# Plachtaa/FAcodec

Measured on AMD Instinct MI355X. Metric: 24kHz audio sec encoded+decoded per wall-sec, higher is better.
Workload: dtype f32; 1 GPU; configs[1]: batch=32/GPU x 2 s @ 24 kHz, forward encoder->FVQ(6 codebooks)->decoder, FAcodec configs/config.yml model (137.7 M params), weights formula-generated, weight-norm re-materialised every step; clips_per_gpu=32, samples_per_clip=48000, parallelism=dp1 (independent clips, no collective)

## Files before the change

### facodec_amd/_lib.py

```python
import ctypes as C
import os

_HERE = os.path.dirname(os.path.abspath(__file__))
LIB_PATH = os.environ.get("FAC_LIB_PATH", os.path.join(_HERE, "libfacodec_hip.so"))

PAD_ZERO, PAD_REFLECT = 0, 1
ACT_NONE, ACT_TANH, ACT_MISH, ACT_LOG_MEL = 0, 1, 2, 3
ACT_GATE, ACT_WN_RES_SKIP = 4, 5

_p = C.c_void_p
_i = C.c_int
_i64 = C.c_int64
_f = C.c_float


class ConvDesc(C.Structure):
    _fields_ = [
        ("x", _p), ("w", _p), ("bias", _p), ("alpha_in", _p), ("alpha_out", _p), ("res", _p), ("y", _p), ("y2", _p), ("alpha_y2", _p), ("w_k1", _p), ("bias_k1", _p),
        ("x_bs", _i64), ("x_cs", _i64), ("y_bs", _i64), ("y_cs", _i64),
        ("B", C.c_int32), ("C_in", C.c_int32), ("T_in", C.c_int32), ("C_out", C.c_int32),
        ("C_out_pad", C.c_int32), ("T_out", C.c_int32),
        ("K", C.c_int32), ("stride", C.c_int32), ("dilation", C.c_int32), ("pad_left", C.c_int32),
        ("pad_mode", C.c_int32), ("n_phase", C.c_int32), ("y_tstride", C.c_int32), ("phase_shift", C.c_int32),
        ("act", C.c_int32),
# ... 211 lines not shown
    "fac_glu_residual": (_i, [_p, _p, _p, _i, _i, _i, _p]),
    "fac_add": (_i, [_p, _p, _p, _i64, _p]),
    "fac_sub2": (_i, [_p, _p, _p, _p, _i64, _p]),
    "fac_mul_mask": (_i, [_p, _p, _i, _i, _i, _p]),
    "fac_wn_res_skip": (_i, [_p, _p, _p, _i, _i, _i, _i, _p]),
    "fac_attention": (_i, [_p, _p, _p, _p, _p, _i, _i, _i, _i, _p]),
    "fac_attention_stream": (_i, [_p, _p, _p, _p, _p, _i, _i, _i, _i, _p]),
    "fac_attention_route": (_i, [_i, _i]),
    "fac_attention_form": (_i, [_i, _i]),
    "fac_attention_tiled_fits": (_i, [_i, _i]),
    "fac_attention_tiled": (_i, [_p, _p, _p, _p, _p, _i, _i, _i, _i, _p]),
    "fac_attention_serial": (_i, [_p, _p, _p, _p, _p, _i, _i, _i, _i, _p]),
    "fac_attention_stream_tile": (_i, [_i]),
    "fac_masked_mean": (_i, [_p, _p, _p, _i, _i, _i, _p]),
    "fac_layernorm_c_affine": (_i, [_p, _p, _p, _i, _i, _i, _p]),
    "fac_stft_frames": (_i, [_p, _p, _i, _i, _i, _i, _i, _i, _i, _p]),
    "fac_stft_frames_ragged": (_i, [_p, _p, _p, _i, _i, _i, _i, _i, _i, _i, _p]),
    "fac_mask_tail": (_i, [_p, _p, _i, _i, _i, _i, _p]),
    "fac_mask_tail_i64": (_i, [_p, _p, _i, _i, _i, _i, _p]),
    "fac_edge_tail": (_i, [_p, _p, _i, _i, _i, _i, _i, _i, _p]),
    "fac_frame_mask": (_i, [_p, _p, _p, _i, _i, _i, _p]),
    "fac_resample": (_i, [C.POINTER(ResampleDesc), _p]),
    "fac_resample_form": (_i, [C.POINTER(ResampleDesc), _p]),
    "fac_kweight_ws_bytes": (_i64, [_i, _i]),
    "fac_kweight_energy": (_i, [C.POINTER(KweightDesc), _p]),
    "fac_loudness_chunk": (_i, [_i]),
    "fac_loudness_gate": (_i, [_p, _i64, _p, _i64, _i, _i, _p, _i, _p, _p, _i, _p]),
    "fac_loudness_gain": (_i, [_p, _i64, _p, _p, _p, _p, C.c_double, _i, _p, _i64, _p, _i, _i, _p]),
    "fac_si_sdr_ws_bytes": (_i64, [_i, _i]),
    "fac_si_sdr": (_i, [_p, _i64, _p, _i64, _p, _p, _p, _i64, _i, _i, _p]),
# ... 49 lines not shown
```

### facodec_amd/csrc/common.h

```cpp
#pragma once
#include <hip/hip_runtime.h>
#include <stdint.h>
#include <stdio.h>
#include <stdarg.h>
#include "../../include/facodec_hip.h"

namespace fac {

void set_error(const char* fmt, ...);

inline int check_launch(const char* what) {
  hipError_t e = hipGetLastError();
  if (e != hipSuccess) {
    set_error("%s: launch failed: %s", what, hipGetErrorString(e));
    return FAC_ERR_LAUNCH;
  }
  return FAC_OK;
}

#define FAC_REQUIRE(cond, ...)          \
  do {                                  \
    if (!(cond)) {                      \
      ::fac::set_error(__VA_ARGS__);    \
      return FAC_ERR_ARG;               \
// ... 57 lines not shown
}
__device__ __forceinline__ f32x2 snake_apply2(f32x2 x, float alpha, float inv) { return x + inv * sin_sq2(alpha * x); }

__device__ __attribute__((noinline)) float apply_act_slow(float v, int act) {
  if (act == FAC_ACT_TANH) return tanhf(v);
  if (act == FAC_ACT_MISH) {
    const float sp = v > 20.f ? v : log1pf(expf(v));
    return v * tanhf(sp);
  }
  if (act == FAC_ACT_LOG_MEL) return (logf(1e-5f + v) + 4.0f) / 4.0f;
  return v;
}

__device__ __forceinline__ float sigmoid_f(float x) { return __fdiv_rn(1.0f, 1.0f + expf(-x)); }

__device__ __forceinline__ int reflect_index(int t, int T, int Text) {
  int j;
  if (t < 0) j = -t;
  else if (t < Text) j = t;
  else j = 2 * (Text - 1) - t;
  return (j >= 0 && j < T) ? j : -1;
}


typedef __bf16 bf16x8 __attribute__((ext_vector_type(8)));
typedef __bf16 bf16x4 __attribute__((ext_vector_type(4)));
typedef float f32x16 __attribute__((ext_vector_type(16)));
typedef float f32x4 __attribute__((ext_vector_type(4)));
typedef unsigned u32x4 __attribute__((ext_vector_type(4)));

// ... 76 lines not shown
```

### facodec_amd/csrc/conv1d_api.hip

```cpp
#include "conv1d_mfma.h"
#include <stdlib.h>

namespace fac {

enum ConvKernel : int {
  CK_128x32 = 0,
  CK_32x256 = 1,
  CK_64x128 = 2,
  CK_96x128 = 3,
  CK_128x128 = 4,
  CK_128x256 = 5,
  CK_96x256 = 6,
  CK_FUSED_RU = 7,
  CK_128x160 = 8,
  CK_NARROW = 9,
  CK_SKINNY = 10,
  CK_BSPLIT = 11,
  CK_CIN1 = 12,
  CK_THIN = 13,
  CK_PW = 14,
  CK_GSPLIT = 15,
  CK_BSPLIT2 = 16,
  CK_PWS = 17,
  CK_PWT = 18,
// ... 73 lines not shown
  {
    long long last = (long long)(d->T_out - 1) * d->stride + (long long)conv_max_tap_offset(a) - d->pad_left;
    int pad_right = last >= d->T_in ? (int)(last - d->T_in + 1) : 0;
    int max_pad = d->pad_left > pad_right ? d->pad_left : pad_right;
    a.T_ext = d->T_in > max_pad ? d->T_in : max_pad + 1;
  }
  if (d->x_p8 || d->y2_p8) {
    const bool gs = d->w_split && (d->K <= 2 || (d->stride > 1 && d->K <= 2 * d->stride)) && conv_gsplit_ok(a) &&
                    !conv_skinny_ok(a, d->ws, d->ws_bytes) && d->C_in % 8 == 0 && d->x_p8_plane_bytes < (1ll << 32);
    const bool ok = !d->y2_p8 && (gs || (d->w_split && !conv_two_level(a) && (d->split_rows == 96 ? conv_bsplit96_p8_ok(a) : conv_bsplit_p8_ok(a)) &&
                                       !conv_cin1_ok(a)));
    FAC_REQUIRE(ok, "conv1d: P8 operands given but the launch does not run on a kernel that takes them (K=%d stride=%d C_in=%d columns=%lld)",
                d->K, d->stride, d->C_in, (long long)d->B * d->T_out);
  }
  if (d->act == FAC_ACT_GATE || d->act == FAC_ACT_WN_RES_SKIP) {
    FAC_REQUIRE(d->w && !d->w_k1 && !d->x_p8 && !conv_two_level(a) && conv_skinny_ok(a, d->ws, d->ws_bytes),
                "conv1d: FAC_ACT_GATE / FAC_ACT_WN_RES_SKIP exist only for few-column launches (B * T_out <= 640) with a workspace");
    k = CK_SKINNY;
    return FAC_OK;
  }
  if (d->w_k1) { k = CK_FUSED_RU; return FAC_OK; }
  a.gflat = 0;
  a.grt = 0;
  if (d->w_split && (a.KV == 9 || a.KV == 3) && d->C_out <= 32 && conv_bsplit2_ok(a)) {
    a.w = reinterpret_cast<const float*>(d->w_split);
    k = CK_BSPLIT2;
    return FAC_OK;
  }
  FAC_REQUIRE(!conv_two_level(a) || d->w, "conv1d: two-level taps outside the split kernel's shapes need fp32 weights");
  const bool pw_on = pw_enabled();
  if (pw_on && d->pw_split && d->w && conv_pwt_ok(a)) { k = CK_PWT; return FAC_OK; }
  if (d->w_split && (d->K <= 2 || (d->stride > 1 && d->K <= 2 * d->stride)) && conv_gsplit_ok(a) &&
      !conv_skinny_ok(a, d->ws, d->ws_bytes)) {
    a.w = reinterpret_cast<const float*>(d->w_split);
    k = CK_GSPLIT;
// ... 108 lines not shown
```

### facodec_amd/csrc/conv1d_bsplit.hip

```cpp
#include "conv1d_bsplit_kernel.h"

namespace fac {

__device__ __forceinline__ void pack_conv_split_body(const float* __restrict__ v, const float* __restrict__ scale,
                                                     bf16x8* __restrict__ out, int C_out, int C_in, int K, int G, int H, int n_st,
                                                     int CO, long long n, int vb, int vg) {
  for (long long idx = (long long)vb * 256 + threadIdx.x; idx < n; idx += (long long)vg * 256) {
    const int co = (int)(idx % CO);
    long long r = idx / CO;
    const int hs = (int)(r % H);
    r /= H;
    const int s = (int)(r % n_st);
    const int ct = (int)(r / n_st);
    const int g = hs % G, k = hs / G;
    const int cog = ct * CO + co;
    const float sc = (scale != nullptr && cog < C_out) ? scale[cog] : 1.0f;
    bf16x8 h, m, l;
#pragma unroll
    for (int i = 0; i < 8; ++i) {
      const int ci = (s * G + g) * 8 + i;
      float w = 0.f;
      if (cog < C_out && ci < C_in && k < K) {
        w = v[((long long)cog * C_in + ci) * K + k];
        if (scale != nullptr) w = __fmul_rn(w, sc);
      }
      __bf16 a, b2, c;
      split3(w, a, b2, c);
      h[i] = a; m[i] = b2; l[i] = c;
    }
    const long long base = ((long long)ct * n_st + s) * 3;
    out[((base + 0) * H + hs) * CO + co] = h;
    out[((base + 1) * H + hs) * CO + co] = m;
    out[((base + 2) * H + hs) * CO + co] = l;
  }
}

__global__ __launch_bounds__(256) void pack_conv_split_kernel(const float* __restrict__ v, const float* __restrict__ scale,
                                                              bf16x8* __restrict__ out, int C_out, int C_in, int K, int G, int H,
                                                              int n_st, int CO, long long n) {
  pack_conv_split_body(v, scale, out, C_out, C_in, K, G, H, n_st, CO, n, blockIdx.x, gridDim.x);
}

__global__ __launch_bounds__(256) void bsplit_batch_kernel(const PrepJob* __restrict__ jobs, const int* __restrict__ first, int njobs) {
  const int j = prep_find_job(first, njobs, blockIdx.x);
  const PrepJob& J = jobs[j];
  pack_conv_split_body(static_cast<const float*>(J.a), static_cast<const float*>(J.b), static_cast<bf16x8*>(J.out), J.i[0], J.i[1],
                       J.i[2], J.i[3], J.i[4], J.i[5], J.i[6], J.n, blockIdx.x - first[j], J.nblocks);
}

int prep_launch_bsplit(const PrepJob* jobs, const int* first, int njobs, int total, hipStream_t s) {
  hipLaunchKernelGGL(bsplit_batch_kernel, dim3(total), dim3(256), 0, s, jobs, first, njobs);
  return check_launch("bsplit_batch");
}

bool conv_bsplit_ok(const ConvArgs& a) {
  if (!((a.K == 7 || a.K == 5 || a.K == 3) && a.stride == 1 && a.n_phase == 1 && a.phase_shift == 0 && a.y_tstride == 1 && !a.alpha_in &&
        !a.w1 && !a.w_batched && (long long)a.B * a.T_out > 640))
    return false;
  const int G = bs_group(a.C_in), tt = G == 2 ? 256 : 512;
  const int kp = G == 2 ? a.K - 1 : ((a.K + 1) & ~1) - 1;
  return a.C_in % (8 * G) == 0 && G * ((tt + kp * a.dil + 63) / 64) <= BS_NSW * BS_XU &&
         a.x_cs * (long long)a.C_in < (1ll << 31);
// ... 13 lines not shown

}

extern "C" int fac_debug_bsplit_occupancy(int lds_bytes) {
  int n = -1;
  auto kern = fac::conv1d_bsplit_kernel<7, 2, 4, fac::BS_NSW_WIDE>;
  (void)hipFuncSetAttribute(reinterpret_cast<const void*>(kern), hipFuncAttributeMaxDynamicSharedMemorySize, (int)fac::FAC_LDS_MAX);
  if (hipOccupancyMaxActiveBlocksPerMultiprocessor(&n, kern, (4 + fac::BS_NSW) * 64, (size_t)lds_bytes) != hipSuccess) return -1;
  return n;
}

static bool split_rows_ok(int K, int rows) { return rows == fac::BS_CO || (rows == fac::BS96_CO && K == 7); }

extern "C" int64_t fac_conv_w_split_rows_bytes(int C_out, int C_in, int K, int rows) {
  using namespace fac;
  if (!split_rows_ok(K, rows)) return -1;
  const int G = rows == BS96_CO ? 1 : bs_group(C_in);
  const int64_t n_ct = (C_out + rows - 1) / rows, n_st = (C_in + 8 * G - 1) / (8 * G);
  return n_ct * n_st * 3 * bs_slots(K, G) * rows * 16;
}

extern "C" int64_t fac_conv_w_split_bytes(int C_out, int C_in, int K) { return fac_conv_w_split_rows_bytes(C_out, C_in, K, fac::BS_CO); }

extern "C" int fac_pack_conv_w_split_rows(const float* v, const float* scale, void* out, int C_out, int C_in, int K, int rows,
                                          fac_stream_t stream) {
  using namespace fac;
  FAC_REQUIRE(v && out && C_out > 0 && C_in > 0 && K > 0, "pack_conv_w_split: bad arguments");
  FAC_REQUIRE(split_rows_ok(K, rows), "pack_conv_w_split: no %d-row tile for K=%d", rows, K);
  const int G = rows == BS96_CO ? 1 : bs_group(C_in);
  const int n_ct = (C_out + rows - 1) / rows, n_st = (C_in + 8 * G - 1) / (8 * G), H = bs_slots(K, G);
  const long long n = (long long)n_ct * n_st * H * rows;
  const int blocks = (int)((n + 255) / 256 < 65535 ? (n + 255) / 256 : 65535);
  if (prep_recording()) {
    PrepJob j{}; j.a = v; j.b = scale; j.out = out; j.kind = PK_CONV_SPLIT; j.nblocks = blocks; j.n = n;
    j.i[0] = C_out; j.i[1] = C_in; j.i[2] = K; j.i[3] = G; j.i[4] = H; j.i[5] = n_st; j.i[6] = rows;
    return prep_record(PU_BSPLIT, j);
  }
  hipLaunchKernelGGL(pack_conv_split_kernel, dim3(blocks), dim3(256), 0, (hipStream_t)stream, v, scale,
                     reinterpret_cast<bf16x8*>(out), C_out, C_in, K, G, H, n_st, rows, n);
  return check_launch("pack_conv_w_split");
}

extern "C" int fac_pack_conv_w_split(const float* v, const float* scale, void* out, int C_out, int C_in, int K,
                                     fac_stream_t stream) {
  return fac_pack_conv_w_split_rows(v, scale, out, C_out, C_in, K, fac::BS_CO, stream);
}
```

### facodec_amd/csrc/conv1d_bsplit_kernel.h

```cpp
#pragma once
#include "conv1d_mfma.h"
#include <type_traits>
#include "inflight_regs.h"
#include "prep_batch.h"

namespace fac {

constexpr int BS_CO = 64;
constexpr int BS96_CO = 96;
constexpr int BS_NSW = 4;
constexpr int BS_NSW_WIDE = 4;
constexpr int BS_XU = 3;
constexpr int BS_WIDE_MIN = 64;
__host__ __device__ constexpr int bs_group(int C_in) { return C_in >= BS_WIDE_MIN ? 2 : 1; }

__host__ __device__ constexpr int bs_slots(int K, int G) { return (G * K + 1) & ~1; }

struct EpiRow {
  float bs, al, inv, a2, i2;
};
__device__ __forceinline__ EpiRow epi_row_load(bool valid, int co, const float* bias, const float* alpha, const float* alpha2) {
  EpiRow r = {0.f, 0.f, 0.f, 0.f, 0.f};
  if (valid) {
    if (bias) r.bs = bias[co];
// ... 448 lines not shown
  {
    const KArgP e = fresh_args();
    const float* tile = reinterpret_cast<const float*>(epi_base);
    constexpr int EP = BS_TT + 4;
    constexpr int NTH = (NMW + NSW) * 64;
    constexpr int QPR = BS_TT / 4;
    float* yg = e->y ? e->y + (long long)b * e->y_bs : nullptr;
    float* y2g = e->y2 ? e->y2 + (long long)b * e->y_bs : nullptr;
    const float* rg = e->res ? e->res + (long long)b * e->y_bs : nullptr;
    const bool vec_ok = (e->y_cs & 3) == 0 && (e->y_bs & 3) == 0 && (!yg || (reinterpret_cast<unsigned long long>(e->y) & 15) == 0) &&
                        (!y2g || (reinterpret_cast<unsigned long long>(e->y2) & 15) == 0) &&
                        (!rg || (reinterpret_cast<unsigned long long>(e->res) & 15) == 0);
    static_assert(QPR % 16 == 0 && NTH % 16 == 0 && (CO * QPR) % 64 == 0 && (CO * QPR + NTH - 1) / NTH <= 16, "EpiRow: 16 lanes share a row, <= 16 iterations");
    const int row_l = (tid + NTH * (lane & 15)) / QPR;
    const EpiRow mine = epi_row_load(row_l < CO && co0 + row_l < e->C_out, co0 + row_l, e->bias, e->alpha_out, y2g ? e->alpha2 : nullptr);
    int j = 0;
    for (int q = tid; q < CO * QPR; q += NTH, ++j) {
      const float bs = epi_row_get(mine.bs, lane, j), al = epi_row_get(mine.al, lane, j), inv = epi_row_get(mine.inv, lane, j);
      float a2 = 0.f, i2 = 0.f;
      if (y2g) { a2 = epi_row_get(mine.a2, lane, j); i2 = epi_row_get(mine.i2, lane, j); }
      const int row = q / QPR, tq = q - row * QPR;
      const int co = co0 + row, t = t0 + 4 * tq;
      if (co >= e->C_out || t >= e->T_out) continue;
      const float4 av = *reinterpret_cast<const float4*>(tile + row * EP + 4 * tq);
      f32x2 v[2] = {{av.x, av.y}, {av.z, av.w}};
      const long long o = (long long)co * e->y_cs + t;
      const bool full = vec_ok && t + 3 < e->T_out;
      float rv[4] = {0.f, 0.f, 0.f, 0.f};
      if (rg) {
        if (full) {
// ... 16 lines not shown
#pragma unroll
        for (int i = 0; i < 2; ++i) w[i] = snake_apply2(v[i], a2, i2);
      }
      if (full) {
        if (yg) *reinterpret_cast<float4*>(yg + o) = make_float4(v[0].x, v[0].y, v[1].x, v[1].y);
        if (y2g) *reinterpret_cast<float4*>(y2g + o) = make_float4(w[0].x, w[0].y, w[1].x, w[1].y);
      } else {
#pragma unroll
        for (int i = 0; i < 4; ++i) {
          if (t + i >= e->T_out) continue;
          if (yg) yg[o + i] = v[i >> 1][i & 1];
          if (y2g) y2g[o + i] = w[i >> 1][i & 1];
        }
      }
    }
  }
  first = !overlap;
  if (vb + (int)gridDim.x < n_tiles) __syncthreads();
  }
  };
  if (wave >= NMW) {
    if constexpr (WIDE) {
      if (a.x_p8 != nullptr) walk(std::integral_constant<int, 2>{});
      else walk(std::integral_constant<int, 1>{});
    } else {
      walk(std::integral_constant<int, 1>{});
    }
  } else {
    walk(std::integral_constant<int, 0>{});
  }
// ... 32 lines not shown
```

### facodec_amd/csrc/misc.hip

```cpp
#include "common.h"
#include <string.h>

namespace fac {

static thread_local char g_err[512] = "";

void set_error(const char* fmt, ...) {
  va_list ap;
  va_start(ap, fmt);
  vsnprintf(g_err, sizeof(g_err), fmt, ap);
  va_end(ap);
}

constexpr int EW_THREADS = 256;
inline int ew_grid(long long n, int per_thread = 1) {
  long long g = (n + (long long)EW_THREADS * per_thread - 1) / ((long long)EW_THREADS * per_thread);
  if (g > 8192) g = 8192;
  if (g < 1) g = 1;
  return (int)g;
}

__global__ void snake_kernel(const float* __restrict__ x, const float* __restrict__ alpha,
                             float* __restrict__ y, int C, int T, long long n) {
  for (long long i = (long long)blockIdx.x * blockDim.x + threadIdx.x; i < n;
// ... 307 lines not shown
  if (tv) {
    const float var = ((red[1][0][lane] + red[1][1][lane]) + (red[1][2][lane] + red[1][3][lane])) / (float)C;
    rstd = __fdiv_rn(1.0f, sqrtf(var + 1e-5f));
    if (wave == 0) {
      stat[0][lane] = mean;
      stat[1][lane] = rstd;
    }
  }
  __syncthreads();
  const float* gm = style + (long long)b * 2 * C;
  float* ob = out + (long long)b * C * T;
  for (int i = tid; i < C * T; i += 256) {
    const int c = i / T, tt = i - c * T;
    const float nv = __fmul_rn(xs[i] - stat[0][tt], stat[1][tt]);
    ob[i] = __fadd_rn(__fmul_rn(nv, gm[c]), gm[C + c]);
  }
}

__global__ void stft_frames_kernel(const float* __restrict__ wave, float* __restrict__ frames, int T,
                                   int n_win, int n_frames, int hop, int pad, int n_off,
                                   long long n) {
  const long long per_b = (long long)n_win * n_frames;
  for (long long i = (long long)blockIdx.x * blockDim.x + threadIdx.x; i < n;
       i += (long long)gridDim.x * blockDim.x) {
    const long long b = i / per_b;
    const long long r = i - b * per_b;
    const int nn = (int)(r / n_frames);
    const int f = (int)(r - (long long)nn * n_frames);
    int t = f * hop + nn + n_off - pad;
    if (t < 0) t = -t;
// ... 218 lines not shown
    const float k = r > 0.f ? scale / ((float)M * r) : 0.f;
    for (int m = 0; m < M; ++m) {
      const float bv = pb[(long long)m * T];
      const float d = logf(fabsf(pa[(long long)m * T]) + eps) - logf(fabsf(bv) + eps);
      const float sg = bv > 0.f ? 1.f : (bv < 0.f ? -1.f : 0.f);
      const float g = -k * d * sg / (fabsf(bv) + eps);
      pd[(long long)m * T] = accumulate ? pd[(long long)m * T] + g : g;
    }
  }
}

}

using namespace fac;

extern "C" int fac_version(void) { return 5; }
extern "C" const char* fac_last_error(void) { return fac::g_err; }

#define EW_LAUNCH(kern, n, ...)                                                         \
  hipLaunchKernelGGL(kern, dim3(ew_grid(n)), dim3(EW_THREADS), 0, (hipStream_t)stream, __VA_ARGS__)

extern "C" int fac_snake_fwd(const float* x, const float* alpha, float* y, int B, int C, int T,
                             fac_stream_t stream) {
  FAC_REQUIRE(x && alpha && y && B > 0 && C > 0 && T > 0, "snake_fwd: bad arguments");
  const long long n = (long long)B * C * T;
  if (T >= 1024 && (long long)B * C <= 65535) {
    hipLaunchKernelGGL(snake_rows_kernel, dim3((T + 1023) / 1024, B * C), dim3(256), 0, (hipStream_t)stream, x, alpha, y, C, T);
  } else {
    EW_LAUNCH(snake_kernel, n, x, alpha, y, C, T, n);
  }
  return check_launch("snake_fwd");
// ... 92 lines not shown
  if (stage_v) lds = lds_v;
  allow_dynamic_lds<attention_kernel>();
  dim3 grid((T + 15) / 16, n_heads, B);
  hipLaunchKernelGGL(attention_kernel, grid, dim3(256), lds, (hipStream_t)stream, q, k, v, mask, out,
                     n_heads, dk, T, stage_v);
  return check_launch("attention");
}

extern "C" int fac_masked_mean(const float* x, const float* mask, float* out, int B, int C, int T,
                               fac_stream_t stream) {
  FAC_REQUIRE(x && out && B > 0 && C > 0 && T > 0, "masked_mean: bad arguments");
  hipLaunchKernelGGL(masked_mean_kernel, dim3(C, B), dim3(64), 0, (hipStream_t)stream, x, mask, out, C, T);
  return check_launch("masked_mean");
}

extern "C" int fac_layernorm_c_affine(const float* x, const float* style, float* out, int B, int C,
                                      int T, fac_stream_t stream) {
  FAC_REQUIRE(x && style && out && B > 0 && C > 0 && T > 0, "layernorm_c_affine: bad arguments");
  if (T <= 8 && (size_t)C * T * 4 <= 64 * 1024) {
    hipLaunchKernelGGL(layernorm_c_small_t_kernel, dim3(B), dim3(256), (size_t)C * T * 4, (hipStream_t)stream, x,
                       style, out, C, T);
    return check_launch("layernorm_c_affine(small T)");
  }
  hipLaunchKernelGGL(layernorm_c_kernel, dim3((T + 63) / 64, B), dim3(256), 0, (hipStream_t)stream, x,
                     style, out, C, T);
  return check_launch("layernorm_c_affine");
}

extern "C" int fac_stft_frames(const float* wave, float* frames, int B, int T, int n_win,
                               int n_frames, int hop, int pad, int n_off, fac_stream_t stream) {
  FAC_REQUIRE(wave && frames && B > 0 && T > 0 && n_win > 0 && n_frames > 0 && hop > 0,
              "stft_frames: bad arguments");
  FAC_REQUIRE(pad < T, "stft_frames: reflect pad %d needs a signal longer than %d samples", pad, T);
  const long long n = (long long)B * n_win * n_frames;
  EW_LAUNCH(stft_frames_kernel, n, wave, frames, T, n_win, n_frames, hop, pad, n_off, n);
  return check_launch("stft_frames");
}

extern "C" int fac_spec_power(const float* spec, float* out, int B, int F, int n_frames, int power,
                              fac_stream_t stream) {
  FAC_REQUIRE(spec && out && B > 0 && F > 0 && n_frames > 0 && (power == 1 || power == 2),
// ... 120 lines not shown
```

### facodec_amd/layers.py

```python
import math

import torch
from torch import nn

from . import ops


def _uniform_(t, bound):
    with torch.no_grad():
        return t.uniform_(-bound, bound)


class ConvWeights(nn.Module):

    def __init__(self, c_in, c_out, k, weight_norm=True, transposed=False, stride=1, bias=True):
        super().__init__()
        self.c_in, self.c_out, self.k = c_in, c_out, k
        self.transposed, self.stride, self.weight_norm = transposed, stride, weight_norm
        shape = (c_in, c_out, k) if transposed else (c_out, c_in, k)
        fan_in = (c_out if transposed else c_in) * k
        w = _uniform_(torch.empty(shape), 1.0 / math.sqrt(fan_in))
        if weight_norm:
            self.weight_g = nn.Parameter(w.reshape(shape[0], -1).norm(dim=1).reshape(shape[0], 1, 1))
            self.weight_v = nn.Parameter(w)
        else:
            self.weight = nn.Parameter(w)
        self.bias = nn.Parameter(_uniform_(torch.empty(c_out), 1.0 / math.sqrt(fan_in))) if bias else None
        self._packed = None
        self._split = None
        self._rows = None
        self._rows_split = None
        self.freeze_packed = False

    def _vg(self):
        return (self.weight_v.detach(), self.weight_g.detach()) if self.weight_norm else (self.weight.detach(), None)

    def _cached(self, slot, pack, *a, **kw):
        cur = getattr(self, slot)
        if cur is None or not self.freeze_packed:
            cur = pack(*self._vg(), *a, out=cur[0] if isinstance(cur, tuple) else cur, **kw)
            setattr(self, slot, cur)
        return cur

    def packed(self):
# ... 1 lines not shown
            return self._cached("_packed", ops.pack_convtr_weight, self.stride)
        return self._cached("_packed", ops.pack_conv_weight)

    def packed_rows(self):
        return self._cached("_rows", ops.pack_convtr_weight_rows, self.stride)

    def packed_rows_split(self):
        return self._cached("_rows_split", ops.pack_convtr_weight_rows_split, self.stride)

    def packed_split_strided(self, stride):
        return self._cached("_split", ops.pack_gemm_weight_split, in_stride=stride)

    def packed_split(self, rows=64):
        return self._cached("_split", ops.pack_conv_weight_split, rows=rows)

    def _apply(self, fn, *a, **kw):
        self._packed = None
        self._split = None
        self._rows = None
        self._rows_split = None
        return super()._apply(fn, *a, **kw)


class _Norm(nn.Module):

    def __init__(self, name, weights):
        super().__init__()
        setattr(self, name, weights)


FLAT_SHORT_CLIPS = True
FLAT_STRIDE1 = True

# ... 21 lines not shown
    def plan(self, B, T, alpha_in=False, plain=True, res=False):
        return ops.plan_conv(self.w.c_out, self.w.c_in, self.kernel_size, self.stride, self.dilation, B, T, -(-T // self.stride),
                             alpha_in=alpha_in, plain=plain, res=res, causal_reflect=self.causal and self.pad_mode == ops.PAD_REFLECT,
                             grad=torch.is_grad_enabled(), c_out_mult16=False, tail="always", flat_infer=FLAT_SHORT_CLIPS,
                             flat_stride1=FLAT_STRIDE1)

    def edge_rule(self):
        if self.causal:
            return None
        if self.stride != 1:
            raise NotImplementedError(f"a non-causal strided SConv1d (k = {self.kernel_size}, stride {self.stride}) pads its right "
                                      "side by an amount that depends on the clip's length: no per-clip edge rule")
        n = ((self.kernel_size - 1) * self.dilation) // 2
        return (n, self.pad_mode) if n > 0 else None

    def run(self, x, alpha_in=None, alpha_out=None, res=None, act=ops.ACT_NONE, alpha_y2=None, want_y=True, edge=None):
        w, k, s_ = self.w, self.kernel_size, self.stride
        write_edge(self, x, edge)
        B, _, T = x.shape
        plan = self.plan(B, T, alpha_in is not None, alpha_out is None and res is None and act == ops.ACT_NONE, res is not None)
        split = (w.packed_split_strided(s_) if plan.layout == ops.W_GEMM_STRIDED
                 else w.packed_split(ops.tile_rows(w.c_out, w.c_in, k)) if plan.layout == ops.W_TAPS
                 else w.packed_split() if plan.layout == ops.W_GEMM else None)
        if plan.form != ops.PER_CLIP:
            P = (k - 1) * self.dilation + 1 - s_
            return ops.conv1d_flat(torch.nn.functional.pad(x, (P, 0), mode="reflect"), split, w.c_out, k, s_, T // s_,
                                   dilation=self.dilation, bias=w.bias, p8=plan.p8, alpha_out=alpha_out, act=act, alpha_y2=alpha_y2,
                                   want_y=want_y)
        x = ops.p8_prepass(x, plan.p8)
        return ops.conv1d(x, w.packed() if split is None else None, w.c_out, k, bias=w.bias,
                          stride=s_, dilation=self.dilation, pad_mode=self.pad_mode, alpha_in=alpha_in,
                          alpha_out=alpha_out, res=res, act=act, causal=self.causal, alpha_y2=alpha_y2, want_y=want_y,
                          w_split=split)

    def forward(self, x):
        return self.run(x)


class SConvTranspose1d(nn.Module):

    def __init__(self, in_channels, out_channels, kernel_size, stride=1, causal=False, norm="none"):
        super().__init__()
        self.convtr = _Norm("convtr", ConvWeights(in_channels, out_channels, kernel_size, norm == "weight_norm",
                                                  transposed=True, stride=stride))
        self.stride = stride
        self.causal = causal

    @property
# ... 79 lines not shown
```

### facodec_amd/ops.py

```python
import ctypes as C
import math
import os
from collections import namedtuple

import torch

from . import _lib
from .wprep import prepared
from .convplan import *
from ._lib import ConvDesc, VqDesc, VqDecodeDesc, ResampleDesc, PAD_REFLECT, PAD_ZERO, ACT_NONE, ACT_TANH, ACT_MISH, ACT_LOG_MEL, ACT_GATE, ACT_WN_RES_SKIP


def pad32(n):
    return (n + 31) & ~31


def cin_pad(c):
    return ((c + 47) // 48) * 48


_RAW_STREAM = getattr(torch._C, "_cuda_getCurrentRawStream", None)
_GET_DEVICE = getattr(torch._C, "_cuda_getDevice", None)


# ... 341 lines not shown
    return out


@prepared
def pack_convtr_weight_rows_split(v, g, stride, out=None):
    rows = pack_convtr_weight_rows(v, g, stride)
    cip, _, R = rows.shape
    c_in = v.shape[0]
    lib = _lib.load()
    nbytes = lib.fac_gemm_w_split_bytes(R, c_in, 2, 1)
    if out is None:
        out = torch.empty(nbytes, device=v.device, dtype=torch.uint8)
    _lib.check(lib.fac_pack_gemm_w_split(_ptr(rows), 1, 2 * R, R, None, out.data_ptr(), R, c_in, 2, 1, _stream()),
               "fac_pack_gemm_w_split(convtr rows)")
    return out, R


@prepared
def pack_conv_weight_split(v, g=None, out=None, scale=None, rows=None):
    v = _dev(v, "weight")
    c_out, c_in, k = v.shape
    if k <= 2:
        return pack_gemm_weight_split(v, g, out=out, scale=scale)
    lib = _lib.load()
    if scale is None and g is not None:
        scale = wn_scale(v, g)
    if rows is None:
        rows = tile_rows(c_out, c_in, k)
    nbytes = lib.fac_conv_w_split_rows_bytes(c_out, c_in, k, rows)
    if nbytes < 0:
# ... 119 lines not shown
    if out is not None and (out.stride(0), out.stride(1)) != (d.y_bs, d.y_cs) and out.shape[0] * out.shape[1] > 1:
        assert out.stride(2) == 1 and y2 is None and res is None and out.shape == (B, c_y, t_out)
        d.y_bs, d.y_cs = out.stride(0), out.stride(1)
    if gate_cond is not None:
        if not (gate_cond.is_cuda and gate_cond.dtype == torch.float32 and gate_cond.dim() == 2 and gate_cond.shape == (B, c_out)
                and (gate_cond.stride(1) == 1 or c_out == 1)):
            raise ValueError(f"gate_cond must be a float32 GPU tensor (B={B}, c_out={c_out}) with contiguous rows, "
                             f"got {tuple(gate_cond.shape)} {gate_cond.dtype} {gate_cond.device}")
        d.gate_cond, d.gate_cond_bs = gate_cond.data_ptr(), gate_cond.stride(0)
    _launch_conv(d, "fac_conv1d_fwd")
    return (out, y2) if alpha_y2 is not None else out


STREAM_FOLD = True
SKINNY_MAX_COLS = 640


def convtr_desc(B, c_in, t_in, c_out, stride, c_out_pad, causal=True, has_history=False, rows=False, split=False):
    t_cols = t_in - 1 if has_history else t_in
    t_total = t_cols * stride
    d = ConvDesc()
    d.x_bs, d.x_cs = c_in * t_in, t_in
    d.y_bs, d.y_cs = c_out * t_total, t_total
    d.B, d.C_in, d.T_in, d.C_out, d.C_out_pad, d.T_out = B, c_in, t_in, c_out, c_out_pad, t_cols
    d.K, d.stride, d.dilation, d.pad_left, d.pad_mode = 2, 1, 1, (0 if has_history else 1), PAD_ZERO
    d.n_phase, d.y_tstride, d.act, d.w_batched, d.w_bs = stride, stride, ACT_NONE, 0, 0
    d.phase_shift = 0 if causal else stride - stride // 2
    if rows or split:
        if not causal or has_history:
            raise _lib.FacodecHipError("the all-phases ConvTranspose1d launch is causal and offline only")
# ... 558 lines not shown
    if kernel in ("lds", "serial") and attention_route(dk, T) != "lds":
        raise _lib.FacodecHipError(f"attention: T={T} too long for the LDS score tile at dk={dk}")
    name = {"stream": "fac_attention_stream", "serial": "fac_attention_serial"}.get(kernel, "fac_attention")
    _lib.check(getattr(_lib.load(), name)(_ptr(q), _ptr(k), _ptr(v), _ptr(mask), _ptr(out), B, n_heads, dk, T, _stream()), name)
    return out


def masked_mean(x, mask):
    x = _dev(x)
    B, c, T = x.shape
    out = torch.empty(B, c, device=x.device, dtype=torch.float32)
    _lib.check(_lib.load().fac_masked_mean(_ptr(x), _ptr(mask), _ptr(out), B, c, T, _stream()), "fac_masked_mean")
    return out


def layernorm_c_affine(x, style):
    x, style = _dev(x), _dev(style)
    B, c, T = x.shape
    out = torch.empty_like(x)
    _lib.check(_lib.load().fac_layernorm_c_affine(_ptr(x), _ptr(style), _ptr(out), B, c, T, _stream()),
               "fac_layernorm_c_affine")
    return out


def stft_frames(wave, n_win, n_frames, hop, pad, n_off):
    wave = _dev(wave, "wave")
    B, T = wave.shape
    frames = torch.empty(B, n_win, n_frames, device=wave.device, dtype=torch.float32)
    _lib.check(_lib.load().fac_stft_frames(_ptr(wave), _ptr(frames), B, T, n_win, n_frames, hop, pad, n_off, _stream()),
               "fac_stft_frames")
    return frames


def _lens(lens, B):
    if not isinstance(lens, torch.Tensor) or not lens.is_cuda:
# ... 916 lines not shown
```

### facodec_amd/quantize.py

```python
import math
import os

import numpy as np
import torch
from torch import nn

from . import dsp, ops
from .wprep import cached_forward
from .layers import ConvWeights, SConv1d, _uniform_


class _Codebook(nn.Module):
    def __init__(self, size, dim):
        super().__init__()
        self.weight = nn.Parameter(torch.randn(size, dim))


class VectorQuantize(nn.Module):

    def __init__(self, input_dim, codebook_size, codebook_dim):
        super().__init__()
        if codebook_dim != 8:
            raise NotImplementedError("the VQ kernel is specialised for codebook_dim = 8 (modules/commons.py:303)")
        self.codebook_size, self.codebook_dim, self.input_dim = codebook_size, codebook_dim, input_dim
# ... 109 lines not shown
            self.cond_layer = SConv1d(gin_channels, 2 * hidden_channels * n_layers, 1, norm="weight_norm")
        for i in range(n_layers):
            self.in_layers.append(SConv1d(hidden_channels, 2 * hidden_channels, kernel_size,
                                          dilation=dilation_rate ** i, norm="weight_norm", causal=causal))
            rs = 2 * hidden_channels if i < n_layers - 1 else hidden_channels
            self.res_skip_layers.append(SConv1d(hidden_channels, rs, 1, norm="weight_norm", causal=causal))

    def forward(self, x, x_mask=None, g=None, edge=None):
        x = x.clone()
        out = torch.zeros_like(x)
        cond = None
        if g is not None:
            cond = self.cond_layer.run(g.reshape(g.shape[0], -1, 1)).reshape(g.shape[0], -1)
        H2 = 2 * self.hidden_channels
        for i in range(self.n_layers):
            a = self.in_layers[i].run(x, edge=edge)
            acts = ops.gate_tanh_sigmoid(a, None if cond is None else cond[:, i * H2:(i + 1) * H2])
            rs = self.res_skip_layers[i].run(acts)
            ops.wn_res_skip_(rs, x, out, last=(i == self.n_layers - 1))
        return out


class _PlainConv(nn.Module):

    def __init__(self, c_in, c_out, k):
        super().__init__()
        b = 1.0 / math.sqrt(c_in * k)
        self.weight = nn.Parameter(_uniform_(torch.empty(c_out, c_in, k), b))
        self.bias = nn.Parameter(_uniform_(torch.empty(c_out), b))
        self.c_in, self.c_out, self.k = c_in, c_out, k

    def plan(self, B, T):
        return ops.plan_conv(self.c_out, self.c_in, self.k, 1, 1, B, T, T, c_out_mult16=False, floor_k=(3, 5, 7), tail=None)

# ... 419 lines not shown
```

### include/facodec_hip.h

```cpp
#ifndef FACODEC_HIP_H
#define FACODEC_HIP_H

#include <stdint.h>

#ifdef __cplusplus
extern "C" {
#endif

typedef void* fac_stream_t;

#define FAC_OK 0
#define FAC_ERR_ARG (-1)
#define FAC_ERR_LAUNCH (-2)

#define FAC_PAD_ZERO 0
#define FAC_PAD_REFLECT 1

#define FAC_ACT_NONE 0
#define FAC_ACT_TANH 1
#define FAC_ACT_MISH 2
#define FAC_ACT_LOG_MEL 3
#define FAC_ACT_GATE 4
#define FAC_ACT_WN_RES_SKIP 5

// ... 49 lines not shown
  int32_t row_phases;
  const void* x_p8;
  int64_t x_p8_plane_bytes;
  void* y2_p8;
  int64_t y2_p8_plane_bytes;
  int32_t pw_split;
  int32_t split_rows;
  const float* gate_cond;
  int64_t gate_cond_bs;
  int32_t keep_tile160;
} fac_conv_desc;

int fac_conv1d_fwd(const fac_conv_desc* d, fac_stream_t stream);
int fac_to_p8(const float* x, const float* alpha, void* out, int B, int C, int T, fac_stream_t stream);
int64_t fac_conv_w_split_bytes(int C_out, int C_in, int K);
int64_t fac_conv_w_split_rows_bytes(int C_out, int C_in, int K, int rows);
int fac_pack_conv_w_split_rows(const float* v, const float* scale, void* out, int C_out, int C_in, int K, int rows, fac_stream_t stream);
int fac_pack_conv_w_split(const float* v, const float* scale, void* out, int C_out, int C_in, int K,
                          fac_stream_t stream);
int64_t fac_conv_w_split2_bytes(int C_out, int C_in, int K, int K1);
int fac_pack_conv_w_split2(const float* v, const float* scale, void* out, int C_out, int C_in, int K, int K1, fac_stream_t stream);
int64_t fac_gemm_w_split_bytes(int R, int C_in, int K, int in_stride);
int fac_pack_gemm_w_split(const float* v, int64_t row_stride, int64_t ci_stride, int64_t k_stride, const float* row_scale, void* out,
                          int R, int C_in, int K, int in_stride, fac_stream_t stream);
int fac_conv1d_variant(const fac_conv_desc* d, char* name, int name_len);

int fac_snake_fwd(const float* x, const float* alpha, float* y, int B, int C, int T,
                  fac_stream_t stream);


// ... 228 lines not shown
int fac_attention_route(int dk, int T);
#define FAC_ATTN_FORM_TILED 0
#define FAC_ATTN_FORM_SERIAL 1
#define FAC_ATTN_FORM_STREAM 2
int fac_attention_form(int dk, int T);
int fac_attention_tiled_fits(int dk, int T);
int fac_attention_tiled(const float* q, const float* k, const float* v, const float* mask, float* out,
                        int B, int n_heads, int dk, int T, fac_stream_t stream);
int fac_attention_serial(const float* q, const float* k, const float* v, const float* mask, float* out,
                         int B, int n_heads, int dk, int T, fac_stream_t stream);
int fac_attention_stream_tile(int which);
int fac_masked_mean(const float* x, const float* mask, float* out, int B, int C, int T,
                    fac_stream_t stream);
int fac_layernorm_c_affine(const float* x, const float* style, float* out, int B, int C, int T,
                           fac_stream_t stream);


int fac_stft_frames(const float* wave, float* frames, int B, int T, int n_win, int n_frames,
                    int hop, int pad, int n_off, fac_stream_t stream);


int fac_stft_frames_ragged(const float* wave, const int32_t* lens, float* frames, int B, int T, int n_win, int n_frames,
                           int hop, int pad, int n_off, fac_stream_t stream);
int fac_mask_tail(float* x, const int32_t* lens, int B, int C, int T, int unit, fac_stream_t stream);
int fac_mask_tail_i64(int64_t* x, const int32_t* lens, int B, int C, int T, int unit, fac_stream_t stream);
int fac_edge_tail(float* x, const int32_t* lens, int B, int C, int T, int mul, int n, int mode, fac_stream_t stream);
int fac_frame_mask(const int32_t* lens, float* mask, int32_t* n_valid, int B, int F, int unit, fac_stream_t stream);
int fac_spec_power(const float* spec, float* out, int B, int F, int n_frames, int power,
                   fac_stream_t stream);
int fac_reduce_pair(const float* a, const float* b, float* out, float* scratch, int64_t n,
// ... 109 lines not shown
```

Before: 1269 audio-s/s.

## Fuse WaveNet tanh-sigmoid gate into conv epilogue; add 16-frame layernorm tiles

Packs the WaveNet in_layer conv weights in a paired row order, so each 64-row output tile holds 32 tanh rows and their 32 matching sigmoid rows. The bsplit epilogue can then apply bias, the conditioning add and the tanh*sigmoid gate directly, which removes the separate gate kernel and its round trip of the 2H pre-activation through global memory. It also adds a layernorm kernel over 16-frame tiles, used by default when the 64-frame grid would launch few blocks, to raise parallelism. The risks are an extra packed weight copy per layer, a slow noinline tanhf/sigmoid path in the epilogue, and a new layernorm reduction order.

Result: no change. 1268 audio-s/s (-0.1%).

```diff
diff --git a/facodec_amd/_lib.py b/facodec_amd/_lib.py
--- a/facodec_amd/_lib.py
+++ b/facodec_amd/_lib.py
@@ -249,6 +249,7 @@
     "fac_attention_stream_tile": (_i, [_i]),
     "fac_masked_mean": (_i, [_p, _p, _p, _i, _i, _i, _p]),
     "fac_layernorm_c_affine": (_i, [_p, _p, _p, _i, _i, _i, _p]),
+    "fac_layernorm_c_affine_form": (_i, [_p, _p, _p, _i, _i, _i, _i, _p]),
     "fac_stft_frames": (_i, [_p, _p, _i, _i, _i, _i, _i, _i, _i, _p]),
     "fac_stft_frames_ragged": (_i, [_p, _p, _p, _i, _i, _i, _i, _i, _i, _i, _p]),
     "fac_mask_tail": (_i, [_p, _p, _i, _i, _i, _i, _p]),
diff --git a/facodec_amd/csrc/common.h b/facodec_amd/csrc/common.h
--- a/facodec_amd/csrc/common.h
+++ b/facodec_amd/csrc/common.h
@@ -95,6 +95,8 @@
 
 __device__ __forceinline__ float sigmoid_f(float x) { return __fdiv_rn(1.0f, 1.0f + expf(-x)); }
 
+__device__ __attribute__((noinline)) float gate_pair_slow(float ta, float sa) { return __fmul_rn(tanhf(ta), sigmoid_f(sa)); }
+
 __device__ __forceinline__ int reflect_index(int t, int T, int Text) {
   int j;
   if (t < 0) j = -t;
diff --git a/facodec_amd/csrc/conv1d_api.hip b/facodec_amd/csrc/conv1d_api.hip
--- a/facodec_amd/csrc/conv1d_api.hip
+++ b/facodec_amd/csrc/conv1d_api.hip
@@ -111,11 +111,23 @@
                 d->K, d->stride, d->C_in, (long long)d->B * d->T_out);
   }
   if (d->act == FAC_ACT_GATE || d->act == FAC_ACT_WN_RES_SKIP) {
+    if (d->act == FAC_ACT_GATE && d->w_split && (d->split_rows & FAC_SPLIT_ROWS_PAIRED)) {
+      FAC_REQUIRE(d->split_rows == (64 | FAC_SPLIT_ROWS_PAIRED) && !d->w_k1 && !d->x_p8 && !conv_two_level(a) && conv_bsplit_ok(a) &&
+                      !conv_cin1_ok(a) && d->C_out % 64 == 0 && !d->alpha_out && !d->res && !d->y2 && !d->y2_p8 && d->y,
+                  "conv1d: FAC_ACT_GATE on paired split weights needs a stride-1 K = 3 / 5 / 7 launch of more than 640 columns with "
+                  "C_in %% 16 == 0, C_out %% 64 == 0, fp32 input and y alone (K=%d stride=%d C_in=%d C_out=%d columns=%lld)",
+                  d->K, d->stride, d->C_in, d->C_out, (long long)d->B * d->T_out);
+      a.w = reinterpret_cast<const float*>(d->w_split);
+      k = CK_BSPLIT;
+      return FAC_OK;
+    }
     FAC_REQUIRE(d->w && !d->w_k1 && !d->x_p8 && !conv_two_level(a) && conv_skinny_ok(a, d->ws, d->ws_bytes),
-                "conv1d: FAC_ACT_GATE / FAC_ACT_WN_RES_SKIP exist only for few-column launches (B * T_out <= 640) with a workspace");
+                "conv1d: FAC_ACT_GATE / FAC_ACT_WN_RES_SKIP exist only for few-column launches (B * T_out <= 640) with a workspace, "
+                "FAC_ACT_GATE also for K = 3 / 5 / 7 launches on paired split weights");
     k = CK_SKINNY;
     return FAC_OK;
   }
+  FAC_REQUIRE(!(d->split_rows & FAC_SPLIT_ROWS_PAIRED), "conv1d: split weights in the paired row order fit the FAC_ACT_GATE launch only");
   if (d->w_k1) { k = CK_FUSED_RU; return FAC_OK; }
   a.gflat = 0;
   a.grt = 0;
diff --git a/facodec_amd/csrc/conv1d_bsplit.hip b/facodec_amd/csrc/conv1d_bsplit.hip
--- a/facodec_amd/csrc/conv1d_bsplit.hip
+++ b/facodec_amd/csrc/conv1d_bsplit.hip
@@ -4,7 +4,7 @@
 
 __device__ __forceinline__ void pack_conv_split_body(const float* __restrict__ v, const float* __restrict__ scale,
                                                      bf16x8* __restrict__ out, int C_out, int C_in, int K, int G, int H, int n_st,
-                                                     int CO, long long n, int vb, int vg) {
+                                                     int CO, int pair, long long n, int vb, int vg) {
   for (long long idx = (long long)vb * 256 + threadIdx.x; idx < n; idx += (long long)vg * 256) {
     const int co = (int)(idx % CO);
     long long r = idx / CO;
@@ -13,7 +13,7 @@
     const int s = (int)(r % n_st);
     const int ct = (int)(r / n_st);
     const int g = hs % G, k = hs / G;
-    const int cog = ct * CO + co;
+    const int cog = !pair ? ct * CO + co : (co < 32 ? ct * 32 + co : (C_out >> 1) + ct * 32 + (co - 32));
     const float sc = (scale != nullptr && cog < C_out) ? scale[cog] : 1.0f;
     bf16x8 h, m, l;
 #pragma unroll
@@ -37,15 +37,15 @@
 
 __global__ __launch_bounds__(256) void pack_conv_split_kernel(const float* __restrict__ v, const float* __restrict__ scale,
                                                               bf16x8* __restrict__ out, int C_out, int C_in, int K, int G, int H,
-                                                              int n_st, int CO, long long n) {
-  pack_conv_split_body(v, scale, out, C_out, C_in, K, G, H, n_st, CO, n, blockIdx.x, gridDim.x);
+                                                              int n_st, int CO, int pair, long long n) {
+  pack_conv_split_body(v, scale, out, C_out, C_in, K, G, H, n_st, CO, pair, n, blockIdx.x, gridDim.x);
 }
 
 __global__ __launch_bounds__(256) void bsplit_batch_kernel(const PrepJob* __restrict__ jobs, const int* __restrict__ first, int njobs) {
   const int j = prep_find_job(first, njobs, blockIdx.x);
   const PrepJob& J = jobs[j];
   pack_conv_split_body(static_cast<const float*>(J.a), static_cast<const float*>(J.b), static_cast<bf16x8*>(J.out), J.i[0], J.i[1],
-                       J.i[2], J.i[3], J.i[4], J.i[5], J.i[6], J.n, blockIdx.x - first[j], J.nblocks);
+                       J.i[2], J.i[3], J.i[4], J.i[5], J.i[6], J.i[7], J.n, blockIdx.x - first[j], J.nblocks);
 }
 
 int prep_launch_bsplit(const PrepJob* jobs, const int* first, int njobs, int total, hipStream_t s) {
@@ -89,6 +89,10 @@
 
 extern "C" int64_t fac_conv_w_split_rows_bytes(int C_out, int C_in, int K, int rows) {
   using namespace fac;
+  if (rows & FAC_SPLIT_ROWS_PAIRED) {
+    if (rows != (BS_CO | FAC_SPLIT_ROWS_PAIRED) || C_out % 64 != 0) return -1;
+    rows = BS_CO;
+  }
   if (!split_rows_ok(K, rows)) return -1;
   const int G = rows == BS96_CO ? 1 : bs_group(C_in);
   const int64_t n_ct = (C_out + rows - 1) / rows, n_st = (C_in + 8 * G - 1) / (8 * G);
@@ -101,6 +105,13 @@
                                           fac_stream_t stream) {
   using namespace fac;
   FAC_REQUIRE(v && out && C_out > 0 && C_in > 0 && K > 0, "pack_conv_w_split: bad arguments");
+  const int pair = (rows & FAC_SPLIT_ROWS_PAIRED) ? 1 : 0;
+  if (pair) {
+    FAC_REQUIRE(rows == (BS_CO | FAC_SPLIT_ROWS_PAIRED) && C_out % 64 == 0,
+                "pack_conv_w_split: the paired row order exists for 64-row tiles and C_out %% 64 == 0 (rows=%d C_out=%d)",
+                rows & ~FAC_SPLIT_ROWS_PAIRED, C_out);
+    rows = BS_CO;
+  }
   FAC_REQUIRE(split_rows_ok(K, rows), "pack_conv_w_split: no %d-row tile for K=%d", rows, K);
   const int G = rows == BS96_CO ? 1 : bs_group(C_in);
   const int n_ct = (C_out + rows - 1) / rows, n_st = (C_in + 8 * G - 1) / (8 * G), H = bs_slots(K, G);
@@ -108,11 +119,11 @@
   const int blocks = (int)((n + 255) / 256 < 65535 ? (n + 255) / 256 : 65535);
   if (prep_recording()) {
     PrepJob j{}; j.a = v; j.b = scale; j.out = out; j.kind = PK_CONV_SPLIT; j.nblocks = blocks; j.n = n;
-    j.i[0] = C_out; j.i[1] = C_in; j.i[2] = K; j.i[3] = G; j.i[4] = H; j.i[5] = n_st; j.i[6] = rows;
+    j.i[0] = C_out; j.i[1] = C_in; j.i[2] = K; j.i[3] = G; j.i[4] = H; j.i[5] = n_st; j.i[6] = rows; j.i[7] = pair;
     return prep_record(PU_BSPLIT, j);
   }
   hipLaunchKernelGGL(pack_conv_split_kernel, dim3(blocks), dim3(256), 0, (hipStream_t)stream, v, scale,
-                     reinterpret_cast<bf16x8*>(out), C_out, C_in, K, G, H, n_st, rows, n);
+                     reinterpret_cast<bf16x8*>(out), C_out, C_in, K, G, H, n_st, rows, pair, n);
   return check_launch("pack_conv_w_split");
 }
 
diff --git a/facodec_amd/csrc/conv1d_bsplit_kernel.h b/facodec_amd/csrc/conv1d_bsplit_kernel.h
--- a/facodec_amd/csrc/conv1d_bsplit_kernel.h
+++ b/facodec_amd/csrc/conv1d_bsplit_kernel.h
@@ -486,6 +486,39 @@
     static_assert(QPR % 16 == 0 && NTH % 16 == 0 && (CO * QPR) % 64 == 0 && (CO * QPR + NTH - 1) / NTH <= 16, "EpiRow: 16 lanes share a row, <= 16 iterations");
     const int row_l = (tid + NTH * (lane & 15)) / QPR;
     const EpiRow mine = epi_row_load(row_l < CO && co0 + row_l < e->C_out, co0 + row_l, e->bias, e->alpha_out, y2g ? e->alpha2 : nullptr);
+    bool gated = false;
+    if constexpr (MB == 2) gated = e->act == FAC_ACT_GATE;
+    if (gated) {
+      const int half = e->C_out >> 1, c0 = co0 >> 1;
+      const float* gc = e->gate_cond ? e->gate_cond + (long long)b * e->gate_cond_bs : nullptr;
+      for (int q = tid; q < 32 * QPR; q += NTH) {
+        const int row = q / QPR, tq = q - row * QPR;
+        const int c = c0 + row, t = t0 + 4 * tq;
+        if (c >= half || t >= e->T_out) continue;
+        const float4 tv = *reinterpret_cast<const float4*>(tile + row * EP + 4 * tq);
+        const float4 sv = *reinterpret_cast<const float4*>(tile + (row + 32) * EP + 4 * tq);
+        const float bt = e->bias ? e->bias[c] : 0.f, bsg = e->bias ? e->bias[half + c] : 0.f;
+        float ta[4] = {tv.x, tv.y, tv.z, tv.w}, sa[4] = {sv.x, sv.y, sv.z, sv.w};
+#pragma unroll
+        for (int i = 0; i < 4; ++i) {
+          ta[i] = __fadd_rn(ta[i] + bt, 0.f);
+          sa[i] = __fadd_rn(sa[i] + bsg, 0.f);
+          if (gc) {
+            ta[i] = __fadd_rn(ta[i], gc[c]);
+            sa[i] = __fadd_rn(sa[i], gc[half + c]);
+          }
+          ta[i] = gate_pair_slow(ta[i], sa[i]);
+        }
+        const long long o = (long long)c * e->y_cs + t;
+        if (vec_ok && t + 3 < e->T_out) {
+          *reinterpret_cast<float4*>(yg + o) = make_float4(ta[0], ta[1], ta[2], ta[3]);
+        } else {
+#pragma unroll
+          for (int i = 0; i < 4; ++i)
+            if (t + i < e->T_out) yg[o + i] = ta[i];
+        }
+      }
+    } else {
     int j = 0;
     for (int q = tid; q < CO * QPR; q += NTH, ++j) {
       const float bs = epi_row_get(mine.bs, lane, j), al = epi_row_get(mine.al, lane, j), inv = epi_row_get(mine.inv, lane, j);
@@ -532,6 +565,7 @@
         }
       }
     }
+    }
   }
   first = !overlap;
   if (vb + (int)gridDim.x < n_tiles) __syncthreads();
diff --git a/facodec_amd/csrc/misc.hip b/facodec_amd/csrc/misc.hip
--- a/facodec_amd/csrc/misc.hip
+++ b/facodec_amd/csrc/misc.hip
@@ -345,6 +345,59 @@
     const int c = i / T, tt = i - c * T;
     const float nv = __fmul_rn(xs[i] - stat[0][tt], stat[1][tt]);
     ob[i] = __fadd_rn(__fmul_rn(nv, gm[c]), gm[C + c]);
+  }
+}
+
+constexpr int LN16_F = 16;
+__global__ __launch_bounds__(256) void layernorm_c_tile16_kernel(const float* __restrict__ x,
+                                                                 const float* __restrict__ style,
+                                                                 float* __restrict__ out, int C, int T) {
+  extern __shared__ float xs[];
+  __shared__ float red[2][4][LN16_F];
+  __shared__ float stat[2][LN16_F];
+  const int tid = threadIdx.x;
+  const int b = blockIdx.y;
+  const int t0 = blockIdx.x * LN16_F;
+  const int nf = T - t0 < LN16_F ? T - t0 : LN16_F;
+  const float* xb = x + (long long)b * C * T + t0;
+  const int n = C * LN16_F;
+  for (int i = tid; i < n; i += 256) {
+    const int c = i >> 4, j = i & 15;
+    xs[i] = j < nf ? xb[(long long)c * T + j] : 0.f;
+  }
+  __syncthreads();
+  const int k = tid >> 4, j = tid & 15;
+  if (tid < 64) {
+    float s = 0.f;
+#pragma unroll 16
+    for (int c = k; c < C; c += 4) s += xs[c * LN16_F + j];
+    red[0][k][j] = s;
+  }
+  __syncthreads();
+  if (tid < 64) {
+    const float mean = ((red[0][0][j] + red[0][1][j]) + (red[0][2][j] + red[0][3][j])) / (float)C;
+    float vs = 0.f;
+#pragma unroll 16
+    for (int c = k; c < C; c += 4) {
+      const float d = xs[c * LN16_F + j] - mean;
+      vs = fmaf(d, d, vs);
+    }
+    red[1][k][j] = vs;
+    if (k == 0) stat[0][j] = mean;
+  }
+  __syncthreads();
+  if (tid < LN16_F) {
+    const float var = ((red[1][0][tid] + red[1][1][tid]) + (red[1][2][tid] + red[1][3][tid])) / (float)C;
+    stat[1][tid] = __fdiv_rn(1.0f, sqrtf(var + 1e-5f));
+  }
+  __syncthreads();
+  const float* gm = style + (long long)b * 2 * C;
+  float* ob = out + (long long)b * C * T + t0;
+  for (int i = tid; i < n; i += 256) {
+    const int c = i >> 4, jj = i & 15;
+    if (jj >= nf) continue;
+    const float nv = __fmul_rn(xs[i] - stat[0][jj], stat[1][jj]);
+    ob[(long long)c * T + jj] = __fadd_rn(__fmul_rn(nv, gm[c]), gm[C + c]);
   }
 }
 
@@ -593,7 +646,7 @@
 
 using namespace fac;
 
-extern "C" int fac_version(void) { return 5; }
+extern "C" int fac_version(void) { return 6; }
 extern "C" const char* fac_last_error(void) { return fac::g_err; }
 
 #define EW_LAUNCH(kern, n, ...)                                                         \
@@ -716,17 +769,30 @@
   return check_launch("masked_mean");
 }
 
-extern "C" int fac_layernorm_c_affine(const float* x, const float* style, float* out, int B, int C,
-                                      int T, fac_stream_t stream) {
-  FAC_REQUIRE(x && style && out && B > 0 && C > 0 && T > 0, "layernorm_c_affine: bad arguments");
-  if (T <= 8 && (size_t)C * T * 4 <= 64 * 1024) {
+extern "C" int fac_layernorm_c_affine_form(const float* x, const float* style, float* out, int B, int C, int T, int form,
+                                           fac_stream_t stream) {
+  FAC_REQUIRE(x && style && out && B > 0 && C > 0 && T > 0 && form >= 0 && form <= 2, "layernorm_c_affine: bad arguments");
+  const size_t lds16 = (size_t)C * LN16_F * 4;
+  FAC_REQUIRE(form != 2 || lds16 <= 128 * 1024, "layernorm_c_affine: the 16-frame tiles hold at most 2048 channels (C=%d)", C);
+  if (form == 0 && T <= 8 && (size_t)C * T * 4 <= 64 * 1024) {
     hipLaunchKernelGGL(layernorm_c_small_t_kernel, dim3(B), dim3(256), (size_t)C * T * 4, (hipStream_t)stream, x,
                        style, out, C, T);
     return check_launch("layernorm_c_affine(small T)");
   }
+  if (form == 2 || (form == 0 && lds16 <= 128 * 1024 && (long long)B * ((T + 63) / 64) < 512)) {
+    allow_dynamic_lds<layernorm_c_tile16_kernel>(128 * 1024);
+    hipLaunchKernelGGL(layernorm_c_tile16_kernel, dim3((T + LN16_F - 1) / LN16_F, B), dim3(256), lds16, (hipStream_t)stream, x,
+                       style, out, C, T);
+    return check_launch("layernorm_c_affine(16-frame tiles)");
+  }
   hipLaunchKernelGGL(layernorm_c_kernel, dim3((T + 63) / 64, B), dim3(256), 0, (hipStream_t)stream, x,
                      style, out, C, T);
   return check_launch("layernorm_c_affine");
+}
+
+extern "C" int fac_layernorm_c_affine(const float* x, const float* style, float* out, int B, int C,
+                                      int T, fac_stream_t stream) {
+  return fac_layernorm_c_affine_form(x, style, out, B, C, T, 0, stream);
 }
 
 extern "C" int fac_stft_frames(const float* wave, float* frames, int B, int T, int n_win,
diff --git a/facodec_amd/layers.py b/facodec_amd/layers.py
--- a/facodec_amd/layers.py
+++ b/facodec_amd/layers.py
@@ -28,6 +28,7 @@
         self.bias = nn.Parameter(_uniform_(torch.empty(c_out), 1.0 / math.sqrt(fan_in))) if bias else None
         self._packed = None
         self._split = None
+        self._split_pair = None
         self._rows = None
         self._rows_split = None
         self.freeze_packed = False
@@ -59,9 +60,13 @@
     def packed_split(self, rows=64):
         return self._cached("_split", ops.pack_conv_weight_split, rows=rows)
 
+    def packed_split_paired(self):
+        return self._cached("_split_pair", ops.pack_conv_weight_split, rows=64 | ops.SPLIT_ROWS_PAIRED)
+
     def _apply(self, fn, *a, **kw):
         self._packed = None
         self._split = None
+        self._split_pair = None
         self._rows = None
         self._rows_split = None
         return super()._apply(fn, *a, **kw)
@@ -113,12 +118,20 @@
         n = ((self.kernel_size - 1) * self.dilation) // 2
         return (n, self.pad_mode) if n > 0 else None
 
-    def run(self, x, alpha_in=None, alpha_out=None, res=None, act=ops.ACT_NONE, alpha_y2=None, want_y=True, edge=None):
+    def gate_fusable(self, B, T):
+        w, k = self.w, self.kernel_size
+        if torch.is_grad_enabled() or self.stride != 1 or w.c_out % 64:
+            return False
+        plan = self.plan(B, T, False, False, False)
+        return plan.layout == ops.W_TAPS and plan.form == ops.PER_CLIP and ops.tile_rows(w.c_out, w.c_in, k) == 64
+
+    def run(self, x, alpha_in=None, alpha_out=None, res=None, act=ops.ACT_NONE, alpha_y2=None, want_y=True, edge=None, gate_cond=None):
         w, k, s_ = self.w, self.kernel_size, self.stride
         write_edge(self, x, edge)
         B, _, T = x.shape
         plan = self.plan(B, T, alpha_in is not None, alpha_out is None and res is None and act == ops.ACT_NONE, res is not None)
         split = (w.packed_split_strided(s_) if plan.layout == ops.W_GEMM_STRIDED
+                 else w.packed_split_paired() if act == ops.ACT_GATE
                  else w.packed_split(ops.tile_rows(w.c_out, w.c_in, k)) if plan.layout == ops.W_TAPS
                  else w.packed_split() if plan.layout == ops.W_GEMM else None)
         if plan.form != ops.PER_CLIP:
@@ -130,7 +143,7 @@
         return ops.conv1d(x, w.packed() if split is None else None, w.c_out, k, bias=w.bias,
                           stride=s_, dilation=self.dilation, pad_mode=self.pad_mode, alpha_in=alpha_in,
                           alpha_out=alpha_out, res=res, act=act, causal=self.causal, alpha_y2=alpha_y2, want_y=want_y,
-                          w_split=split)
+                          w_split=split, gate_cond=gate_cond)
 
     def forward(self, x):
         return self.run(x)
diff --git a/facodec_amd/ops.py b/facodec_amd/ops.py
--- a/facodec_amd/ops.py
+++ b/facodec_amd/ops.py
@@ -379,6 +379,9 @@
     _lib.check(lib.fac_pack_gemm_w_split(_ptr(rows), 1, 2 * R, R, None, out.data_ptr(), R, c_in, 2, 1, _stream()),
                "fac_pack_gemm_w_split(convtr rows)")
     return out, R
+
+
+SPLIT_ROWS_PAIRED = 0x100
 
 
 @prepared
@@ -528,6 +531,7 @@
 
 STREAM_FOLD = True
 SKINNY_MAX_COLS = 640
+WN_FUSED = True
 
 
 def convtr_desc(B, c_in, t_in, c_out, stride, c_out_pad, causal=True, has_history=False, rows=False, split=False):
@@ -1116,11 +1120,18 @@
     return out
 
 
-def layernorm_c_affine(x, style):
+LAYERNORM_TILE16 = True
+LN_FORMS = {None: 0, "tile64": 1, "tile16": 2}
+
+
+def layernorm_c_affine(x, style, form=None):
     x, style = _dev(x), _dev(style)
     B, c, T = x.shape
     out = torch.empty_like(x)
-    _lib.check(_lib.load().fac_layernorm_c_affine(_ptr(x), _ptr(style), _ptr(out), B, c, T, _stream()),
+    f = LN_FORMS[form]
+    if f == 0 and not LAYERNORM_TILE16 and not (T <= 8 and c * T * 4 <= 64 * 1024):
+        f = 1
+    _lib.check(_lib.load().fac_layernorm_c_affine_form(_ptr(x), _ptr(style), _ptr(out), B, c, T, f, _stream()),
                "fac_layernorm_c_affine")
     return out
 
diff --git a/facodec_amd/quantize.py b/facodec_amd/quantize.py
--- a/facodec_amd/quantize.py
+++ b/facodec_amd/quantize.py
@@ -147,10 +147,14 @@
             cond = self.cond_layer.run(g.reshape(g.shape[0], -1, 1)).reshape(g.shape[0], -1)
         H2 = 2 * self.hidden_channels
         for i in range(self.n_layers):
-            a = self.in_layers[i].run(x, edge=edge)
-            acts = ops.gate_tanh_sigmoid(a, None if cond is None else cond[:, i * H2:(i + 1) * H2])
+            last = i == self.n_layers - 1
+            g_i = None if cond is None else cond[:, i * H2:(i + 1) * H2]
+            if ops.WN_FUSED and self.in_layers[i].gate_fusable(x.shape[0], x.shape[2]):
+                acts = self.in_layers[i].run(x, act=ops.ACT_GATE, gate_cond=g_i, edge=edge)
+            else:
+                acts = ops.gate_tanh_sigmoid(self.in_layers[i].run(x, edge=edge), g_i)
             rs = self.res_skip_layers[i].run(acts)
-            ops.wn_res_skip_(rs, x, out, last=(i == self.n_layers - 1))
+            ops.wn_res_skip_(rs, x, out, last=last)
         return out
 
 
diff --git a/include/facodec_hip.h b/include/facodec_hip.h
--- a/include/facodec_hip.h
+++ b/include/facodec_hip.h
@@ -87,6 +87,7 @@
 int fac_conv1d_fwd(const fac_conv_desc* d, fac_stream_t stream);
 int fac_to_p8(const float* x, const float* alpha, void* out, int B, int C, int T, fac_stream_t stream);
 int64_t fac_conv_w_split_bytes(int C_out, int C_in, int K);
+#define FAC_SPLIT_ROWS_PAIRED 0x100
 int64_t fac_conv_w_split_rows_bytes(int C_out, int C_in, int K, int rows);
 int fac_pack_conv_w_split_rows(const float* v, const float* scale, void* out, int C_out, int C_in, int K, int rows, fac_stream_t stream);
 int fac_pack_conv_w_split(const float* v, const float* scale, void* out, int C_out, int C_in, int K,
@@ -345,6 +346,8 @@
                     fac_stream_t stream);
 int fac_layernorm_c_affine(const float* x, const float* style, float* out, int B, int C, int T,
                            fac_stream_t stream);
+int fac_layernorm_c_affine_form(const float* x, const float* style, float* out, int B, int C, int T, int form,
+                                fac_stream_t stream);
 
 
 int fac_stft_frames(const float* wave, float* frames, int B, int T, int n_win, int n_frames,
```
